# RegulatoryGenomicsGroup/chicdiff

Hardware: AMD Instinct MI355X
Metric: interactions/sec NB-GLM Wald test (higher is better)
Workload: dtype f64; 1 GPU; synthetic 2000000 interactions x 8 samples (4v4), size factors + offsets(theta=0.5) + dispersions + Wald, design ~condition; rows_per_gpu=2000000, samples=8, global_rows=2000000, parallelism=rows-sharded x1, collectives=none (single rank), ranks_in_communicator=1

## Files before the change

chicdiff_amd/csrc/api.hip:

```cpp
#include <math.h>
#include <stdarg.h>
#include <stdio.h>
#include <stdlib.h>
#include <string.h>

#include <algorithm>
#include <mutex>
#include <thread>
#include <string>
#include <vector>
#include <unordered_set>

#include <dlfcn.h>

#include "common.h"
#include "philox.h"
#include "prior_mc.h"

using namespace cd;

namespace cd {
struct ChinputCols {
    std::vector<int32_t> bait, oe, N;
    std::string error;
};
int64_t chinput_parse(const char *path, int nthreads, ChinputCols &c);
}

struct KTimer {
    std::string name;
    hipEvent_t e0 = nullptr, e1 = nullptr;
    double ms = 0;
    int launches = 0;
    double bytes = 0;
};

struct HostOpts {
    int select_all_rounds = 0;
    int trend_one_launch_per_pass = 0;
    int sharded_trend_gather = 1;
    int trend_mad_in_kernel = 1;
    int local_trend_substitute = 1;
    int fuse_offsets = 1;
    int theta_grid_concurrency = 5;
    int host_copy_threads = 12;
    int bench_fake_world = 0;
    int fault_inject = 0;
    int region_assemble_generic = 0;
    int chicago_tables_run_merge = 1;
};

struct chicdiff_hip_ctx {
    int device = 0;
    bool no_persistent_trend = false;
    Opts tune{};
    HostOpts host;
    char *tg_buf = nullptr;
    size_t tg_bytes = 0;
    double shard_n[kSelMaxWorld] = {0};
    bool shard_n_valid = false;
    int64_t tg_total = 0;
    double *tg_x = nullptr, *tg_y = nullptr, *tg_resid = nullptr;
    int32_t *tg_flags = nullptr;
    int32_t *h_flag = nullptr;
    FusedOffsets fuse;
    int refits = 0;
    bool sf_overflow_seen = false;
    int32_t *d_carry = nullptr;
    char *io_dev = nullptr, *io_pin = nullptr;
    size_t io_dev_bytes = 0, io_pin_bytes = 0;
    ChinputCols *chin = nullptr;
    struct EarlyCopy {
        int n = 0;
        struct Item { int col; char *pin; size_t bytes; } item[10];
        hipEvent_t ready = nullptr, done = nullptr;
        bool issued = false;
// ... 9 lines not shown
    void *allgather_user = nullptr;
    int world = 1, rank = 0;
    void *rccl_lib = nullptr, *rccl_comm = nullptr;
    int (*rccl_allreduce)(const void *, void *, size_t, int, int, void *, hipStream_t) = nullptr;
    int (*rccl_allgather)(const void *, void *, size_t, int, void *, hipStream_t) = nullptr;
    int (*rccl_comm_destroy)(void *) = nullptr;
    const char *(*rccl_error_string)(int) = nullptr;
    char err[512] = {0};
    int64_t cap_n = 0;
    int cap_S = 0;
    void *ws = nullptr;
    size_t ws_bytes = 0;
    char *aux = nullptr;
    size_t aux_bytes = 0;
    FitWork w{};
    double *d_sf = nullptr;
    double *d_logfact = nullptr;
    PmcTable *d_pmc[4] = {nullptr, nullptr, nullptr, nullptr};
    double *d_nf_tmp = nullptr;
    unsigned int *d_sfhist = nullptr;
    bool sfhist_dirty = false;
    FitScalars *h_sc = nullptr;
    double *h_sf = nullptr;
    int timing = 0;
    std::vector<KTimer> timers;
    std::vector<std::pair<int, hipEvent_t>> pending;
    std::vector<hipEvent_t> event_pool;
    int scope_depth = 0;
    std::unordered_set<void *> user_allocs;
    std::mutex user_mu;
};

static char g_create_err[512];
constexpr int64_t kFuseOffsetsMaxRows = 1 << 18;

static const PmcTable &pmc_table(int df) {
    static PmcTable tables[4];
    static bool ready[4] = {false, false, false, false};
    static std::mutex mu;
    std::lock_guard<std::mutex> lock(mu);
    if (!ready[df]) {
        pmc_build(df, tables[df]);
        ready[df] = true;
    }
    return tables[df];
}

static int fail(chicdiff_hip_ctx *c, int code, const char *fmt, ...) {
    va_list ap;
    va_start(ap, fmt);
    vsnprintf(c ? c->err : g_create_err, 512, fmt, ap);
    va_end(ap);
    return code;
}
#define HIPCHK(c, call)                                                                              \
    do {                                                                                             \
        hipError_t e_ = (call);                                                                      \
        if (e_ != hipSuccess) return fail(c, CHICDIFF_E_HIP, "%s: %s", #call, hipGetErrorString(e_)); \
    } while (0)

extern "C" {

const char *chicdiff_hip_last_error(const chicdiff_hip_ctx *ctx) { return ctx ? ctx->err : g_create_err; }

void chicdiff_hip_default_opts(chicdiff_nbglm_opts *o) {
    o->minDisp = 1e-8;
    o->dispTol = 1e-6;
// ... 3 lines not shown
    o->betaTol = 1e-8;
    o->minmu = 0.5;
    o->outlierSD = 2.0;
    o->dispPriorVar = NAN;
    o->trendCoef[0] = o->trendCoef[1] = NAN;
    o->fitType = 0;
    o->_pad = 0;
}

struct OptionDef {
    const char *name;
    int32_t Opts::*tune;
    int HostOpts::*host;
    int64_t lo, hi, no_lo, no_hi;
};
static const OptionDef kOptions[] = {
    {"line_search_spread", &Opts::spread, nullptr, 0, 3, 1, 0},
    {"line_search_min_waves", &Opts::min_waves, nullptr, 0, 4, 1, 1},
    {"line_search_chunk", &Opts::chunk, nullptr, 0, 64, 1, 7},
    {"line_search_prio", &Opts::prio, nullptr, 0, 100, 1, 0},
    {"line_search_schedule", &Opts::schedule, nullptr, 0, 4, 2, 2},
    {"line_search_deal", &Opts::deal, nullptr, 0, 64, 1, 0},
    {"line_search_classes_a", &Opts::classes_a, nullptr, 0, 6, 1, 0},
    {"line_search_fillers", &Opts::fillers, nullptr, -1, 1, 1, 0},
    {"line_search_filler_stop", &Opts::filler_stop, nullptr, -1, 100, 1, 0},
    {"theta_grid_concurrency", nullptr, &HostOpts::theta_grid_concurrency, 1, 16, 1, 0},
    {"host_copy_threads", nullptr, &HostOpts::host_copy_threads, 1, 64, 1, 0},
    {"select_all_rounds", nullptr, &HostOpts::select_all_rounds, 0, 1, 1, 0},
    {"trend_one_launch_per_pass", nullptr, &HostOpts::trend_one_launch_per_pass, 0, 1, 1, 0},
    {"sharded_trend_gather", nullptr, &HostOpts::sharded_trend_gather, 0, 1, 1, 0},
    {"trend_persistent_blocks", &Opts::trend_blocks, nullptr, 0, 256, 1, 0},
    {"trend_mad_in_kernel", nullptr, &HostOpts::trend_mad_in_kernel, 0, 1, 1, 0},
    {"fuse_offsets", nullptr, &HostOpts::fuse_offsets, 0, 2, 1, 0},
    {"region_assemble_generic", nullptr, &HostOpts::region_assemble_generic, 0, 1, 1, 0},
    {"chicago_tables_run_merge", nullptr, &HostOpts::chicago_tables_run_merge, 0, 1, 1, 0},
    {"fault_inject", nullptr, &HostOpts::fault_inject, 0, 7, 1, 0},
    {"bench_fake_world", nullptr, &HostOpts::bench_fake_world, 0, kGatherMaxWorld, 1, 0},
    {"local_trend_substitute", nullptr, &HostOpts::local_trend_substitute, 0, 1, 1, 0},
};

int chicdiff_hip_set_option(chicdiff_hip_ctx *c, const char *name, int64_t value) {
    if (!c || !name) return CHICDIFF_E_INVALID;
    for (const OptionDef &d : kOptions) {
        if (strcmp(name, d.name) != 0 || value < d.lo || value > d.hi || (value >= d.no_lo && value <= d.no_hi)) continue;
        if (d.host == &HostOpts::bench_fake_world && value > 1 && !getenv("CHICDIFF_BENCH_FAKE_WORLD"))
            return fail(c, CHICDIFF_E_INVALID, "set_option: bench_fake_world is a rehearsal hook of bench.py (CHICDIFF_BENCH_FAKE_WORLD unset)");
        if (d.tune) c->tune.*d.tune = (int32_t)value;
        else c->host.*d.host = (int)value;
        return CHICDIFF_OK;
    }
    return fail(c, CHICDIFF_E_INVALID, "set_option: unknown option or value (%s = %lld)", name, (long long)value);
}

int chicdiff_hip_create(chicdiff_hip_ctx **out, int32_t device) {
    if (!out) return fail(nullptr, CHICDIFF_E_INVALID, "ctx out pointer is NULL");
    *out = nullptr;
    int ndev = 0;
    hipError_t e = hipGetDeviceCount(&ndev);
    if (e != hipSuccess || ndev <= 0)
        return fail(nullptr, CHICDIFF_E_HIP, "no HIP device available (%s): the HIP path cannot run, and there is no CPU fallback",
                    e != hipSuccess ? hipGetErrorString(e) : "device count 0");
    if (device < 0 || device >= ndev) return fail(nullptr, CHICDIFF_E_INVALID, "device %d out of range [0,%d)", device, ndev);
    chicdiff_hip_ctx *c = new chicdiff_hip_ctx();
    c->device = device;
    if ((e = hipSetDevice(device)) != hipSuccess || (e = hipStreamCreateWithFlags(&c->own_stream, hipStreamNonBlocking)) != hipSuccess ||
        (e = hipHostMalloc((void **)&c->h_sc, sizeof(FitScalars))) != hipSuccess ||
// ... 705 lines not shown
    launch_resid_hist(dm, wm, d_hist, c->stream);
    if (!mad_local)
        if (int rc = do_allreduce(c, d_hist, kPmcBins)) return rc;
    const int df = d.S - d.p;
    if (!c->d_pmc[df]) {
        HIPCHK(c, hipMalloc((void **)&c->d_pmc[df], sizeof(PmcTable)));
        HIPCHK(c, hipMemcpy(c->d_pmc[df], &pmc_table(df), sizeof(PmcTable), hipMemcpyHostToDevice));
    }
    launch_prior_mc(d, c->w, d_hist, c->d_pmc[df], c->stream);
    return CHICDIFF_OK;
}

static int read_scalars(chicdiff_hip_ctx *c) {
    HIPCHK(c, hipMemcpyAsync(c->h_sc, c->w.sc, sizeof(FitScalars), hipMemcpyDeviceToHost, c->stream));
    HIPCHK(c, hipStreamSynchronize(c->stream));
    return CHICDIFF_OK;
}

static int fit_pass(chicdiff_hip_ctx *c, const int32_t *d_counts, const double *d_nf, FitDims d, const Opts &o,
                    const chicdiff_nbglm_out *d_out, bool all_rounds) {
    int rc;
    hipStream_t st = c->stream;
    FitWork &w = c->w;
    c->tg_total = 0;
    HIPCHK(c, hipMemsetAsync(w.sc, 0, align256(sizeof(FitScalars)) + kQueueBytes + 1024, st));
    const int world = c->world > 0 ? c->world : 1;
    const bool col_slots = c->allreduce && world <= kSelMaxWorld;
    const size_t slot_doubles = (size_t)(d.S + 1) * 2;
    double *slots = col_slots ? w.hist : nullptr;
    if (col_slots) HIPCHK(c, hipMemsetAsync(slots, 0, sizeof(double) * slot_doubles * world, st));
    {
        Scope t(c, "prep");
        const bool fused = c->fuse.fm != nullptr && d.S <= 16 && d_nf == c->d_nf_tmp;
        launch_prep(d_counts, const_cast<double *>(d_nf), d, w, o, st, fused ? c->fuse : FusedOffsets());
        launch_prep_finish(d, w, col_slots ? slots + slot_doubles * c->rank : nullptr, st);
    }
    if (col_slots) {
        if ((rc = do_allreduce(c, slots, (int64_t)(slot_doubles * world)))) return rc;
    } else if ((rc = do_allreduce(c, w.sc->colsum, kMaxS + 1)))
        return rc;
    if (c->allreduce) launch_xim(d, w, slots, world, st);
    {
        Scope t(c, "disp_gene");
        Opts og = o;
        og.xim_here = c->allreduce ? 0 : 1;
        launch_disp_gene(d_counts, d_nf, d, w, og, st);
    }
    bool mad_in_kernel = false;
    if (o.trendIn[0] == o.trendIn[0] && o.trendIn[1] == o.trendIn[1]) {
        launch_trend_init(d, w, o, st);
        HIPCHK(c, hipMemcpyAsync(w.sc->coefs, o.trendIn, sizeof(double) * 2, hipMemcpyHostToDevice, st));
        HIPCHK(c, hipStreamSynchronize(st));
    } else if (o.fit_type == 1) {
        if (c->allreduce) return fail(c, CHICDIFF_E_INVALID, "fitType \"mean\" is not available for sharded fits");
        std::vector<double> g((size_t)d.n);
        HIPCHK(c, hipMemcpyAsync(g.data(), w.dispGene, sizeof(double) * (size_t)d.n, hipMemcpyDeviceToHost, st));
        HIPCHK(c, hipStreamSynchronize(st));
        size_t m = 0;
        for (size_t i = 0; i < g.size(); i++)
            if (g[i] > 10 * o.minDisp) g[m++] = g[i];
        if (m == 0) return fail(c, CHICDIFF_E_NUMERIC, "fitType \"mean\": no gene-wise estimate above 10 * minDisp");
        const size_t lo = (size_t)floor((double)m * 0.001), hi = m - lo;
        if (lo > 0) {
            std::nth_element(g.begin(), g.begin() + lo, g.begin() + m);
            std::nth_element(g.begin() + lo, g.begin() + (hi - 1), g.begin() + m);
        }
        long double acc = 0;
        for (size_t i = lo; i < hi; i++) acc += g[i];
// ... 123 lines not shown
        } else
            break;
        c->refits++;
    }
    if (scalars) {
        const FitScalars *s = c->h_sc;
        int status = 0;
        if (s->failed) status |= CHICDIFF_ST_TREND_FAILED;
        if (s->trend_local) status |= CHICDIFF_ST_TREND_LOCAL;
        scalars->trendCoef[0] = s->coefs[0];
        scalars->trendCoef[1] = s->coefs[1];
        scalars->varLogDispEsts = s->varLogDispEsts;
        scalars->dispPriorVar = s->dispPriorVar;
        scalars->nAllZero = (int64_t)hs[2];
        scalars->sumDeviance = hs[2] > 0 ? NAN : hs[0];
        scalars->trendOuterIter = s->outer_it;
        if (hs[2] > 0) status |= CHICDIFF_ST_ALLZERO_ROWS;
        if (hs[1] > 0) status |= CHICDIFF_ST_BETA_NONCONV;
        if (prior_by_simulation(d, o)) status |= CHICDIFF_ST_PRIORVAR_MC;
        scalars->status = status;
    }
    return CHICDIFF_OK;
}

static int begin_call(chicdiff_hip_ctx *c, int rc, int64_t n, int32_t S) {
    timing_reset(c);
    if ((rc = shard_consensus(c, rc, n))) return rc;
    HIPCHK(c, hipSetDevice(c->device));
    if ((rc = ensure_workspace(c, n, S))) return rc;
    c->refits = 0;
    return CHICDIFF_OK;
}

static void form_offsets(chicdiff_hip_ctx *c, const double *d_fullMean, int64_t n, int32_t S, double theta, int mix) {
    if (d_fullMean && S <= 16 && c->host.fuse_offsets && (c->host.fuse_offsets == 2 || n <= kFuseOffsetsMaxRows)) {
        c->fuse.fm = d_fullMean;
        c->fuse.sf = c->d_sf;
        c->fuse.theta = theta;
        c->fuse.mix = mix;
    } else {
        Scope t(c, "offsets");
        launch_offsets(d_fullMean, c->d_sf, n, S, theta, mix, c->d_nf_tmp, c->stream);
    }
}

extern "C" {

int chicdiff_hip_nbglm_fit_dev(chicdiff_hip_ctx *c, const int32_t *d_counts, const double *d_nf, int64_t n, int32_t S,
                               const int32_t *group, const chicdiff_nbglm_opts *opts, const chicdiff_nbglm_out *d_out,
                               chicdiff_nbglm_scalars *scalars) {
    if (!c) return CHICDIFF_E_INVALID;
    FitDims d;
    int rc = (!d_counts || !d_nf) ? fail(c, CHICDIFF_E_INVALID, "counts / nf pointer is NULL") : check_counts_group(c, n, S, group, d);
    if (!rc) rc = check_opts(c, opts);
    if ((rc = begin_call(c, rc, n, S))) return rc;
    HIPCHK(c, hipMemsetAsync(c->d_carry, 0, sizeof(int32_t), c->stream));
    rc = fit_dev_impl(c, d_counts, d_nf, d, make_opts(c, opts, S), d_out, scalars, c->host.select_all_rounds != 0);
    timing_collect(c);
    return rc;
}

static int ensure_io(chicdiff_hip_ctx *c, size_t dev_bytes, size_t pin_bytes) {
    if (c->io_dev_bytes < dev_bytes) {
        if (c->io_dev) { HIPCHK(c, hipStreamSynchronize(c->stream)); (void)hipFree(c->io_dev); c->io_dev = nullptr; c->io_dev_bytes = 0; }
        hipError_t e = hipMalloc((void **)&c->io_dev, dev_bytes);
        if (e != hipSuccess) return fail(c, CHICDIFF_E_NOMEM, "device arena of %zu bytes: %s", dev_bytes, hipGetErrorString(e));
        c->io_dev_bytes = dev_bytes;
    }
// ... 1049 lines not shown
```

chicdiff_amd/csrc/common.h:

```cpp
#pragma once
#include <hip/hip_runtime.h>
#include <stdint.h>

#include "../../include/chicdiff_hip.h"
#include "fit_driver.h"
#include "fit_state.h"

namespace cd {

constexpr int kRedBlocks = 1024;

struct FitDims {
    int64_t n;
    int32_t S, p, nA, nB;
    uint64_t gmask;
};

struct FitWork {
    double *baseMean, *baseVar, *gm0, *gm1, *rough, *binit0, *binit1, *crow;
    double *dispGene, *dispFit, *dispMAP, *disp, *beta0, *beta1, *resid;
    int32_t *allZero, *geneIter, *mapIter, *outlier, *betaIter, *optimConv;
    int32_t *order;
    uint8_t *cls;
    int32_t *gridlist;
// ... 87 lines not shown
    if (a == 4) return kSchedMinDispSlot;
    if (a == 5) return (mode == kSchedSix || mode == kSchedMinDispLast) ? kSchedClassesFine - 1 : kSchedMinDispSlot;
    return kSchedClassesFine;
}
#ifdef __HIPCC__
template <int NC>
__device__ __forceinline__ void order_hist_store(const unsigned int (&mine)[NC], unsigned int *hist) {
    __shared__ unsigned int s_cnt[NC];
    if (threadIdx.x < NC) s_cnt[threadIdx.x] = 0;
    __syncthreads();
#pragma unroll
    for (int k = 0; k < NC; k++) {
        unsigned int v = mine[k];
        for (int off = 32; off > 0; off >>= 1) v += __shfl_down(v, off);
        if ((threadIdx.x & 63) == 0 && v) atomicAdd(&s_cnt[k], v);
    }
    __syncthreads();
    if (threadIdx.x < NC) hist[threadIdx.x * kSchedBlocks + blockIdx.x] = s_cnt[threadIdx.x];
}
__device__ __forceinline__ void class_peers(int c, bool valid, int lane, unsigned int &rank, unsigned int &count) {
    unsigned long long m = __ballot(valid);
#pragma unroll
    for (int b = 0; b < 5; b++) {
        const bool bit = (c >> b) & 1;
        const unsigned long long set = __ballot(bit);
        m &= bit ? set : ~set;
    }
    rank = __popcll(m & ((1ull << lane) - 1ull));
    count = __popcll(m);
}
#endif

struct FusedOffsets { const double *fm = nullptr; const double *sf = nullptr; double theta = 0; int mix = 0; };
void launch_prep(const int32_t *counts, double *nf, FitDims d, FitWork w, Opts o, hipStream_t st, FusedOffsets fo = FusedOffsets());
void launch_prep_finish(FitDims d, FitWork w, double *slot, hipStream_t st);
void launch_xim(FitDims d, FitWork w, const double *slots, int world, hipStream_t st);
void launch_disp_gene(const int32_t *counts, const double *nf, FitDims d, FitWork w, Opts o, hipStream_t st);
void launch_order_build(FitDims d, FitWork w, int classesA, bool have_hist, hipStream_t st, bool fine = false);
void launch_disp_map(const int32_t *counts, const double *nf, FitDims d, FitWork w, Opts o, hipStream_t st);
void launch_trend_persistent(FitDims d, FitWork w, Opts o, hipStream_t st, bool with_mad);
int trend_persistent_blocks();
void launch_trend_init(FitDims d, FitWork w, Opts o, hipStream_t st);
int trend_blocks();
void launch_trend_pass(FitDims d, FitWork w, Opts o, hipStream_t st, bool fused_step);
void launch_trend_step(FitDims d, FitWork w, Opts o, hipStream_t st);
constexpr int kLfMaxV = 100;
struct LfVerts { int nv; int _pad; double x[kLfMaxV], f[kLfMaxV], d[kLfMaxV]; };
void launch_lf_hist(FitDims d, FitWork w, Opts o, int use_dist, double xv, uint64_t prefix, int shift, double *hist, hipStream_t st);
void launch_lf_sums(FitDims d, FitWork w, Opts o, double xv, double h, double *partials, double *out8, hipStream_t st);
void launch_lf_eval(FitDims d, FitWork w, const LfVerts &v, hipStream_t st);
void launch_trend_gather(FitDims d, FitWork w, Opts o, double *xg, double *yg, hipStream_t st);
constexpr int kGatherMaxWorld = 64;
struct GatherLayout { int32_t world, _pad; int64_t block, maxn; int64_t off[kGatherMaxWorld + 1]; };
void launch_trend_compact(const GatherLayout &gl, const double *recv, double *xg, double *yg, hipStream_t st);
void launch_poke(int32_t *p, int32_t v, hipStream_t st);
void launch_flag_to_double(const int32_t *flag, double *out, hipStream_t st);
void launch_dispfit_resid(FitDims d, FitWork w, Opts o, hipStream_t st);
void launch_prior_var(FitDims d, FitWork w, Opts o, hipStream_t st);
void launch_resid_hist(FitDims d, FitWork w, double *out40, hipStream_t st);
void launch_prior_mc(FitDims d, FitWork w, const double *hist40, const void *table, hipStream_t st);
void launch_wald_prep(const int32_t *counts, const double *nf, FitDims d, FitWork w, Opts o, hipStream_t st);
void launch_wald_irls(const int32_t *counts, const double *nf, FitDims d, FitWork w, Opts o, hipStream_t st);
void launch_wald_final(const int32_t *counts, const double *nf, FitDims d, FitWork w, Opts o,
                       const chicdiff_nbglm_out &out, hipStream_t st);
void launch_wald_intercept(const int32_t *counts, const double *nf, FitDims d, FitWork w, Opts o,
                           const chicdiff_nbglm_out &out, hipStream_t st);
void launch_dev_sum_finish(FitDims d, FitWork w, const int32_t *carry, const double *sf_dev, hipStream_t st);

// ... 151 lines not shown
```

chicdiff_amd/csrc/devmath.h:

```cpp
#pragma once
#include <hip/hip_runtime.h>

#include "exp_table.h"
#include "fit_state.h"
#include "log_table.h"

namespace cd {

__device__ __forceinline__ double fma3(double a, double b, double c) {
    double d;
    asm("v_fma_f64 %0, %1, %2, %3" : "=v"(d) : "v"(a), "v"(b), "v"(c));
    return d;
}

__device__ __forceinline__ double rcp(double x) {
    double r = __builtin_amdgcn_rcp(x);
    double e = fma(-x, r, 1.0);
    r = fma(r, e, r);
    e = fma(-x, r, 1.0);
    return fma(r, e, r);
}

__device__ __forceinline__ double rcp_or_div(double x) { return (x > 1e-300 && x < 1e300) ? rcp(x) : 1.0 / x; }

// ... 237 lines not shown
        const double temp = y * (xnum + 18154.981253343561249) / (xden + 45507.789335026729956);
        return 2.0 * (0.5 - temp);
    }
    double temp;
    if (y <= 5.656854249492380195206754896838) {
        double xnum = 1.0765576773720192317e-8 * y, xden = y;
        xnum = (xnum + 0.39894151208813466764) * y;  xden = (xden + 22.266688044328115691) * y;
        xnum = (xnum + 8.8831497943883759412) * y;   xden = (xden + 235.38790178262499861) * y;
        xnum = (xnum + 93.506656132177855979) * y;   xden = (xden + 1519.377599407554805) * y;
        xnum = (xnum + 597.27027639480026226) * y;   xden = (xden + 6485.558298266760755) * y;
        xnum = (xnum + 2494.5375852903726711) * y;   xden = (xden + 18615.571640885098091) * y;
        xnum = (xnum + 6848.1904505362823326) * y;   xden = (xden + 34900.952721145977266) * y;
        xnum = (xnum + 11602.651437647350124) * y;   xden = (xden + 38912.003286093271411) * y;
        temp = (xnum + 9842.7148383839780218) / (xden + 19685.429676859990727);
    } else if (y < 37.5193) {
        const double xsq = 1.0 / (y * y);
        double xnum = 0.02307344176494017303 * xsq, xden = xsq;
        xnum = (xnum + 0.21589853405795699) * xsq;      xden = (xden + 1.28426009614491121) * xsq;
        xnum = (xnum + 0.1274011611602473639) * xsq;    xden = (xden + 0.468238212480865118) * xsq;
        xnum = (xnum + 0.022235277870649807) * xsq;     xden = (xden + 0.0659881378689285515) * xsq;
        xnum = (xnum + 0.001421619193227893466) * xsq;  xden = (xden + 0.00378239633202758244) * xsq;
        temp = xsq * (xnum + 2.9112874951168792e-5) / (xden + 7.29751555083966205e-5);
        temp = (0.398942280401432677939946059934 - temp) / y;
    } else {
        return 0.0;
    }
    const double xsq = trunc(y * 16) / 16;
    const double del = (y - xsq) * (y + xsq);
    return 2.0 * (exp(-xsq * xsq * 0.5) * exp(-del * 0.5) * temp);
}


__device__ __forceinline__ double rlog_t(double x, const LogEntry *lt) { return (x > 2.3e-308 && x < 1.7e308) ? tlog(x, lt) : log(x); }
__device__ __forceinline__ void offsets_row16(double (&v)[16], int S, const double *__restrict__ sf, double theta, int mix, const LogEntry *lt) {
    const double iS = 1.0 / S;
    double sl = 0;
#pragma unroll
    for (int j = 0; j < 16; j++)
        if (j < S) sl += rlog_t(v[j], lt);
    const double gmean = exp(sl * iS);
    const double ig = (gmean > 1e-300 && gmean < 1e300) ? rcp(gmean) : 1.0 / gmean;
    bool anyna = false;
#pragma unroll
    for (int j = 0; j < 16; j++)
        if (j < S) {
            v[j] = v[j] * ig;
            anyna |= (v[j] != v[j]);
        }
    double sl2 = 0;
#pragma unroll
    for (int j = 0; j < 16; j++)
        if (j < S) {
            if (anyna) v[j] = sf[j];
            if (mix) {
                v[j] = v[j] * (1 - theta) + sf[j] * theta;
                sl2 += rlog_t(v[j], lt);
            }
        }
    if (mix) {
        const double g2 = exp(sl2 * iS);
        const double i2 = (g2 > 1e-300 && g2 < 1e300) ? rcp(g2) : 1.0 / g2;
#pragma unroll
        for (int j = 0; j < 16; j++)
            if (j < S) v[j] = v[j] * i2;
    }
}

}
```

chicdiff_amd/csrc/disp_kernels.hip:

```cpp
#include <stdio.h>
#include <stdlib.h>

#include <vector>

#include "common.h"
#include "devmath.h"

namespace cd {

struct DD { double hi, lo; };
__device__ __forceinline__ void dd_add(DD &a, double x) {
    const double s = a.hi + x, bb = s - a.hi;
    a.lo += (a.hi - (s - bb)) + (x - bb);
    a.hi = s;
}
__device__ __forceinline__ void dd_add(DD &a, const DD &b) {
    dd_add(a, b.hi);
    a.lo += b.lo;
    const double s = a.hi + a.lo;
    a.lo = a.lo - (s - a.hi);
    a.hi = s;
}

struct CountProfile { unsigned int w0 = 0, w1 = 0, w2 = 0; };
__device__ __forceinline__ void profile_add(CountProfile &c, int y) {
    const unsigned int m = (unsigned int)(y < 10 ? y : 10);
    const unsigned int a = m < 4u ? m : 4u, b = m < 4u ? 0u : (m < 8u ? m - 4u : 4u), d = m < 8u ? 0u : m - 8u;
    c.w0 += 0x01010101u & (a == 4u ? 0xffffffffu : ((1u << (8u * a)) - 1u));
    c.w1 += 0x01010101u & (b == 4u ? 0xffffffffu : ((1u << (8u * b)) - 1u));
    c.w2 += 0x00000101u & ((1u << (8u * d)) - 1u);
}
__device__ __forceinline__ void prep_store(FitDims d, FitWork w, int64_t i, double s, double g0, double g1, double v,
                                           double est, int64_t tot) {
    w.baseMean[i] = s / d.S;
    w.baseVar[i] = v / (d.S - 1);
    w.gm0[i] = g0;
    w.gm1[i] = g1;
    w.rough[i] = fmax(est / (d.S - d.p), 0.0);
    w.allZero[i] = (tot == 0);
}

template <bool FUSED>
__global__ __launch_bounds__(256) void prep16_kernel(const int32_t *__restrict__ counts,
                                                     double *__restrict__ nf, FitDims d, FitWork w, FusedOffsets fo) {
    __shared__ LogEntry s_lt[FUSED ? 64 : 1];
    if (FUSED) log_table_to_lds(s_lt);
    extern __shared__ uint32_t s_tile[];
    __shared__ DD s_part[256];
    __shared__ unsigned char s_live[256];
    const int T = blockDim.x;
    const int64_t n = d.n;
    const int S = d.S;
    const int64_t stride = row_stride(S);
    const int ldw = (int)(stride / 4) + 1, qpr = (int)(stride / 16);
    const int tid = threadIdx.x;
    const int ncol = S + 1, G = T / ncol, cg = tid / ncol, cc = tid % ncol;
    DD colacc{0.0, 0.0};
    for (int64_t base = (int64_t)blockIdx.x * T; base < n; base += (int64_t)gridDim.x * T) {
        const int64_t i = base + tid;
        const int nrows = n - base < T ? (int)(n - base) : T;
        if (i < n) {
            double q[16];
            double s = 0, g0 = 0, g1 = 0;
            int64_t tot = 0;
            int32_t sign = 0;
            CountProfile cprof;
            uint32_t *row = s_tile + tid * ldw;
            row[7] = 0;
            for (int k = 8 + 3 * S; k < (int)(stride / 4); k++) row[k] = 0;
            double fv[16];
            if (FUSED) {
#pragma unroll
                for (int j = 0; j < 16; j++) fv[j] = j < S ? fo.fm[(int64_t)j * n + i] : 1.0;
                offsets_row16(fv, S, fo.sf, fo.theta, fo.mix, s_lt);
#pragma unroll
                for (int j = 0; j < 16; j++)
                    if (j < S) nf[(int64_t)j * n + i] = fv[j];
            }
#pragma unroll
            for (int j = 0; j < 16; j++) {
                q[j] = 0;
                if (j < S) {
                    const int32_t k = counts[(int64_t)j * n + i];
                    const double f = FUSED ? fv[j] : nf[(int64_t)j * n + i];
                    row[8 + 2 * j] = (uint32_t)__double2loint(f);
                    row[8 + 2 * j + 1] = (uint32_t)__double2hiint(f);
                    row[8 + 2 * S + j] = (uint32_t)k;
                    profile_add(cprof, k);
                    sign |= k;
                    q[j] = (double)k / f;
                    tot += k;
                    s += q[j];
                    if ((d.gmask >> j) & 1) g1 += q[j]; else g0 += q[j];
                }
            }
            const double bm = s / S;
            g0 /= d.nA;
            if (d.p == 2) g1 /= d.nB;
            row[0] = (uint32_t)__double2loint(g0);
            row[1] = (uint32_t)__double2hiint(g0) | (tot == 0 ? 0x80000000u : 0u);
            row[2] = (uint32_t)__double2loint(g1);
            row[3] = (uint32_t)__double2hiint(g1);
            row[4] = cprof.w0;
            row[5] = cprof.w1;
            row[6] = cprof.w2;
            s_live[tid] = tot != 0;
            const double m0 = fmax(1.0, g0), m1 = fmax(1.0, g1);
            const double i0 = 1.0 / (m0 * m0), i1 = 1.0 / (m1 * m1);
            double v = 0, est = 0;
#pragma unroll
            for (int j = 0; j < 16; j++)
                if (j < S) {
                    v += (q[j] - bm) * (q[j] - bm);
                    const bool g = (d.gmask >> j) & 1;
                    const double mj = g ? m1 : m0;
                    est += ((q[j] - mj) * (q[j] - mj) - mj) * (g ? i1 : i0);
                }
            prep_store(d, w, i, s, g0, g1, v, est, tot);
            if (sign < 0) w.sc->neg_counts = 1;
        }
        __syncthreads();
        uint4 *dst = reinterpret_cast<uint4 *>(w.rowpack + base * stride);
        for (int c = tid; c < nrows * qpr; c += T) {
            const uint32_t *src = s_tile + (c / qpr) * ldw + (c % qpr) * 4;
            dst[c] = make_uint4(src[0], src[1], src[2], src[3]);
        }
        if (cg < G) {
            DD a{0.0, 0.0};
            for (int r = cg; r < nrows; r += G)
                if (s_live[r]) {
                    const uint32_t *src = s_tile + r * ldw + 8 + 2 * cc;
                    dd_add(a, cc < S ? __hiloint2double((int)src[1], (int)src[0]) : 1.0);
                }
            s_part[cg * ncol + cc] = a;
        }
        __syncthreads();
        if (tid < ncol)
            for (int g = 0; g < G; g++) dd_add(colacc, s_part[g * ncol + tid]);
        __syncthreads();
    }
    if (tid < ncol) {
        w.partials[((int64_t)tid * gridDim.x + blockIdx.x) * 2] = colacc.hi;
        w.partials[((int64_t)tid * gridDim.x + blockIdx.x) * 2 + 1] = colacc.lo;
    }
}

__global__ __launch_bounds__(256) void prep_kernel(const int32_t *__restrict__ counts,
                                                   const double *__restrict__ nf, FitDims d, FitWork w) {
    const int64_t n = d.n;
    const int S = d.S;
    for (int64_t i = blockIdx.x * (int64_t)blockDim.x + threadIdx.x; i < n; i += (int64_t)gridDim.x * blockDim.x) {
        double s = 0, g0 = 0, g1 = 0;
        int64_t tot = 0;
        double *rp_nf = reinterpret_cast<double *>(w.rowpack + i * row_stride(S) + kRowHdr);
        int32_t *rp_y = reinterpret_cast<int32_t *>(rp_nf + S);
        CountProfile cprof;
        for (int j = 0; j < S; j++) {
            const int32_t k = counts[(int64_t)j * n + i];
            if (k < 0) w.sc->neg_counts = 1;
            profile_add(cprof, k);
            rp_nf[j] = nf[(int64_t)j * n + i];
            rp_y[j] = k;
            const double q = (double)k / nf[(int64_t)j * n + i];
            tot += k;
            s += q;
            if ((d.gmask >> j) & 1) g1 += q; else g0 += q;
        }
        const double bm = s / S;
        g0 /= d.nA;
        if (d.p == 2) g1 /= d.nB;
        reinterpret_cast<double2 *>(row_hdr(w.rowpack, i, S))[0] = make_double2(tot == 0 ? -0.0 : g0, g1);
        reinterpret_cast<uint4 *>(row_hdr(w.rowpack, i, S))[1] = make_uint4(cprof.w0, cprof.w1, cprof.w2, 0u);
        const double m0 = fmax(1.0, g0), m1 = fmax(1.0, g1);
        double v = 0, est = 0;
        for (int j = 0; j < S; j++) {
            const double q = (double)counts[(int64_t)j * n + i] / nf[(int64_t)j * n + i];
// ... 30 lines not shown
        for (int off = 32; off > 0; off >>= 1) dd_add(a, DD{__shfl_down(a.hi, off), __shfl_down(a.lo, off)});
    } else {
        double s = 0;
        for (int b = lane; b < nblk; b += 64) s += w.partials[(int64_t)j * nblk + b];
        for (int off = 32; off > 0; off >>= 1) s += __shfl_down(s, off);
        a.hi = s;
    }
    if (lane == 0) {
        if (slot) {
            slot[2 * j] = a.hi;
            slot[2 * j + 1] = a.lo;
        } else {
            const double s = a.hi + a.lo;
            if (j < d.S) w.sc->colsum[j] = s; else w.sc->nnz = s;
        }
    }
}

__global__ void xim_kernel(FitDims d, FitWork w, const double *slots, int world) {
    if (threadIdx.x || blockIdx.x) return;
    if (slots)
        for (int j = 0; j <= d.S; j++) {
            DD a{0.0, 0.0};
            for (int r = 0; r < world; r++) dd_add(a, DD{slots[((size_t)r * (d.S + 1) + j) * 2], slots[((size_t)r * (d.S + 1) + j) * 2 + 1]});
            const double s = a.hi + a.lo;
            if (j < d.S) w.sc->colsum[j] = s; else w.sc->nnz = s;
        }
    double x = 0;
    for (int j = 0; j < d.S; j++) x += 1.0 / (w.sc->colsum[j] / w.sc->nnz);
    w.sc->xim = x / d.S;
}

constexpr int kColsumBlocks = 512;
static int prep16_blocks(int) { return 1024; }
void launch_prep(const int32_t *counts, double *nf, FitDims d, FitWork w, Opts, hipStream_t st, FusedOffsets fo) {
    if (d.S <= 16) {
        const int T = row_stride(d.S) > 128 ? 128 : 256;
        if (fo.fm) prep16_kernel<true><<<prep16_blocks(d.S), T, (size_t)T * (row_stride(d.S) + 4), st>>>(counts, nf, d, w, fo);
        else prep16_kernel<false><<<prep16_blocks(d.S), T, (size_t)T * (row_stride(d.S) + 4), st>>>(counts, nf, d, w, fo);
    } else {
        prep_kernel<<<kRedBlocks, 256, 0, st>>>(counts, nf, d, w);
        colsum_kernel<<<dim3(kColsumBlocks, d.S + 1), 256, 0, st>>>(nf, d, w);
    }
}
void launch_prep_finish(FitDims d, FitWork w, double *slot, hipStream_t st) {
    colsum_finish_kernel<<<d.S + 1, 64, 0, st>>>(d, w, d.S <= 16 ? prep16_blocks(d.S) : kColsumBlocks, d.S <= 16, slot);
}
void launch_xim(FitDims d, FitWork w, const double *slots, int world, hipStream_t st) { xim_kernel<<<1, 64, 0, st>>>(d, w, slots, world); }

constexpr int kSchedClassesA = 2, kSchedDeal = 8;
template <int NC>
__global__ __launch_bounds__(256) void order_hist_kernel(const uint8_t *__restrict__ cls, int64_t n, int64_t tile, unsigned int *hist) {
    const int64_t lo = (int64_t)blockIdx.x * tile, hi = lo + tile < n ? lo + tile : n;
    unsigned int mine[NC] = {};
    for (int64_t i = lo + threadIdx.x; i < hi; i += 256) {
        const int c = cls[i];
#pragma unroll
        for (int k = 0; k < NC; k++) mine[k] += (c == k);
    }
    order_hist_store<NC>(mine, hist);
}
template <int NC>
__global__ __launch_bounds__(256) void order_scatter_kernel(const uint8_t *__restrict__ cls, int64_t n, int64_t tile,
                                                            const unsigned int *__restrict__ hist, int32_t *__restrict__ order,
                                                            FitScalars *sc, int classesA, int classesB) {
    static_assert(NC <= 32 && kSchedBlocks == 4 * 256, "8 threads per class sum 256 partial counts; class_peers() tells 32 classes apart");
    __shared__ unsigned int s_m[NC][256];
    __shared__ unsigned int s_edge[NC];
    __shared__ unsigned int s_part[NC][8][2];
    __shared__ unsigned int s_tot[NC], s_pre[NC];
    __shared__ unsigned int s_wh[4][NC];
    __shared__ unsigned int s_wbase[4][NC];
    const int nblk = gridDim.x, t = threadIdx.x, lane = t & 63, wave = t >> 6, blk = blockIdx.x;
    if (t < 4 * NC) (&s_wh[0][0])[t] = 0;
    __syncthreads();
    const int64_t lo = (int64_t)blk * tile, hi = lo + tile < n ? lo + tile : n;
    const int64_t quarter = tile / 4;
    const int64_t wlo = lo + wave * quarter, whi = wlo + quarter < hi ? wlo + quarter : hi;
    for (int64_t i0 = wlo; i0 < whi; i0 += 64) {
// ... 805 lines not shown
```

chicdiff_amd/csrc/global_kernels.hip:

```cpp
#include "common.h"
#include "devmath.h"
#include "prior_mc.h"

namespace cd {

template <int K>
__device__ __forceinline__ void block_reduce_store(double (&v)[K], double *out) {
    __shared__ double red[K][4];
    const int lane = threadIdx.x & 63, wave = threadIdx.x >> 6;
#pragma unroll
    for (int k = 0; k < K; k++) {
        double x = v[k];
        for (int off = 32; off > 0; off >>= 1) x += __shfl_down(x, off);
        if (lane == 0) red[k][wave] = x;
    }
    __syncthreads();
    if (threadIdx.x < K) out[threadIdx.x] = (red[threadIdx.x][0] + red[threadIdx.x][1]) + (red[threadIdx.x][2] + red[threadIdx.x][3]);
}

__global__ void reduce_partials_kernel(const double *partials, int nblk, int K, double *sums) {
    __shared__ double red[256];
    for (int k = 0; k < K; k++) {
        double acc = 0;
        for (int b = threadIdx.x; b < nblk; b += 256) acc += partials[(int64_t)b * K + k];
// ... 1446 lines not shown
            double rk[2] = {rank0, 0};
            sf_list_select(list, a.n, false, m0, nb, b0, 1, rk, s_h, s_c, &s_nc, s_res);
            rk[0] = rank1;
            sf_list_select(list, a.n, true, m1, nb, b1, 1, rk, s_h, s_c, &s_nc, s_res + 1);
        }
    }
    __syncthreads();
    if (threadIdx.x == 0) {
        sc->sel_prefix[2 * col] = s_res[0];
        sc->sel_prefix[2 * col + 1] = s_res[1];
        if (col == 0) sc->sel_fast_done = 1;
        sel_finish_col(a, sc, col);
    }
}

void launch_sf_direct(const int32_t *counts, int64_t n, int S, SelArgs a, FitWork w, unsigned int *hist, uint64_t *lists,
                      int32_t *clear_flag, int cus, hipStream_t st) {
    const int nb = sf_bins(S);
    int64_t hb = (n + kSfThreads - 1) / kSfThreads;
    if (hb > (cus > 0 ? cus : 256)) hb = cus > 0 ? cus : 256;
    unsigned int *gcnt = hist + kSfHistWords;
    if (S <= 4) sf_hist_kernel<4><<<(unsigned)hb, kSfThreads, 0, st>>>(counts, n, S, nb, hist, clear_flag);
    else if (S <= 8) sf_hist_kernel<8><<<(unsigned)hb, kSfThreads, 0, st>>>(counts, n, S, nb, hist, clear_flag);
    else sf_hist_kernel<16><<<(unsigned)hb, kSfThreads, 0, st>>>(counts, n, S, nb, hist, clear_flag);
    sf_pick_kernel<<<S, kSfThreads, 0, st>>>(w, hist, gcnt, nb);
    if (S <= 4) sf_list_kernel<4><<<(unsigned)hb, kSfThreads, 0, st>>>(counts, n, S, nb, w, gcnt, lists);
    else if (S <= 8) sf_list_kernel<8><<<(unsigned)hb, kSfThreads, 0, st>>>(counts, n, S, nb, w, gcnt, lists);
    else sf_list_kernel<16><<<(unsigned)hb, kSfThreads, 0, st>>>(counts, n, S, nb, w, gcnt, lists);
    sf_finish_kernel<<<S, kSfThreads, 0, st>>>(a, w, nb, gcnt, lists);
}

__device__ __forceinline__ double rlog(double x) { return (x > 0.0 && x < 1.7e308) ? flog(x) : log(x); }

__global__ __launch_bounds__(256) void offsets16_kernel(const double *__restrict__ fm, const double *__restrict__ sf,
                                                        int64_t n, int S, double theta, int mix,
                                                        double *__restrict__ out) {
    __shared__ LogEntry s_lt[64];
    log_table_to_lds(s_lt);
    for (int64_t i = blockIdx.x * 256 + threadIdx.x; i < n; i += (int64_t)gridDim.x * 256) {
        double v[16];
#pragma unroll
        for (int j = 0; j < 16; j++) v[j] = j < S ? fm[(int64_t)j * n + i] : 1.0;
        offsets_row16(v, S, sf, theta, mix, s_lt);
#pragma unroll
        for (int j = 0; j < 16; j++)
            if (j < S) out[(int64_t)j * n + i] = v[j];
    }
}

__global__ __launch_bounds__(256) void offsets_kernel(const double *__restrict__ fm, const double *__restrict__ sf,
                                                      int64_t n, int S, double theta, int mix,
                                                      double *__restrict__ out) {
    for (int64_t i = blockIdx.x * 256 + threadIdx.x; i < n; i += (int64_t)gridDim.x * 256) {
        double sl = 0;
        for (int j = 0; j < S; j++) sl += rlog(fm[(int64_t)j * n + i]);
        const double gmean = exp(sl / S);
        bool anyna = false;
        for (int j = 0; j < S; j++) {
            const double m3 = fm[(int64_t)j * n + i] / gmean;
            anyna |= (m3 != m3);
        }
        double g2 = 1.0;
        if (mix) {
            double sl2 = 0;
            for (int j = 0; j < S; j++) {
                const double m3 = anyna ? sf[j] : fm[(int64_t)j * n + i] / gmean;
                sl2 += rlog(m3 * (1 - theta) + sf[j] * theta);
            }
            g2 = exp(sl2 / S);
        }
        for (int j = 0; j < S; j++) {
            double m3 = anyna ? sf[j] : fm[(int64_t)j * n + i] / gmean;
            if (mix) m3 = (m3 * (1 - theta) + sf[j] * theta) / g2;
            out[(int64_t)j * n + i] = m3;
        }
    }
}
__global__ __launch_bounds__(256) void offsets_sf_kernel(const double *__restrict__ sf, int64_t n, int S, double *__restrict__ out) {
    for (int64_t i = blockIdx.x * 256 + threadIdx.x; i < n; i += (int64_t)gridDim.x * 256)
        for (int j = 0; j < S; j++) out[(int64_t)j * n + i] = sf[j];
}
void launch_offsets(const double *fm, const double *sf_dev, int64_t n, int S, double theta, int mix, double *out,
                    hipStream_t st) {
    int64_t blocks = (n + 255) / 256;
    if (blocks > 4096) blocks = 4096;
    if (!fm) {
        offsets_sf_kernel<<<(unsigned)blocks, 256, 0, st>>>(sf_dev, n, S, out);
        return;
    }
    if (S <= 16)
        offsets16_kernel<<<(unsigned)blocks, 256, 0, st>>>(fm, sf_dev, n, S, theta, mix, out);
    else
        offsets_kernel<<<(unsigned)blocks, 256, 0, st>>>(fm, sf_dev, n, S, theta, mix, out);
}

constexpr int kWinCap = 256 * 12;
__global__ __launch_bounds__(256) void window_sums_kernel(const int32_t *__restrict__ fragN,
                                                          const double *__restrict__ fragFM, int64_t nfrag, int S,
                                                          const int64_t *__restrict__ rptr, int64_t n,
                                                          int32_t *__restrict__ N, double *__restrict__ FM) {
    __shared__ int32_t s_n[kWinCap];
    __shared__ double s_f[kWinCap];
    const int j = blockIdx.y;
    const int64_t nblk = (n + 255) / 256;
    for (int64_t blk = blockIdx.x; blk < nblk; blk += gridDim.x) {
        const int64_t i0 = blk * 256, i1 = (i0 + 256 < n) ? i0 + 256 : n;
        const int64_t f0 = rptr[i0], f1 = rptr[i1];
        const int64_t i = i0 + threadIdx.x;
        const bool staged = (f1 - f0) <= kWinCap;
        int64_t lo = 0, hi = 0;
        if (i < i1) { lo = rptr[i]; hi = rptr[i + 1]; }
        if (staged) {
            __syncthreads();
            const int span = (int)(f1 - f0);
            if (fragN) {
                int32_t v[12];
#pragma unroll
                for (int k = 0; k < 12; k++) {
                    const int e = threadIdx.x + k * 256;
                    v[k] = e < span ? fragN[(int64_t)j * nfrag + f0 + e] : 0;
                }
#pragma unroll
                for (int k = 0; k < 12; k++) {
                    const int e = threadIdx.x + k * 256;
// ... 685 lines not shown
```

Before: 584.8 million interactions/s.

## Specialize prep kernel by sample count, prefetch next rows, size grid to residency

The prep kernel is now templated on padded sample count (4/8/16), so S=8 uses 8-wide register arrays instead of 16. It software-prefetches the next grid-stride iteration's counts and means into registers before the tile store. The grid is sized from occupancy × CU count instead of a fixed 1024 blocks. Fused offset formation is also enabled for all row counts (the 2^18 row cap is removed), the per-block column accumulator moves to shared memory, and the finish kernel receives the actual block count. Together these aim to cut memory latency stalls and the separate offsets pass, at the cost of more registers per thread and more template instantiations.

```diff
diff --git a/chicdiff_amd/csrc/api.hip b/chicdiff_amd/csrc/api.hip
--- a/chicdiff_amd/csrc/api.hip
+++ b/chicdiff_amd/csrc/api.hip
@@ -42,6 +42,7 @@
     int trend_mad_in_kernel = 1;
     int local_trend_substitute = 1;
     int fuse_offsets = 1;
+    int prep_blocks = 0;
     int theta_grid_concurrency = 5;
     int host_copy_threads = 12;
     int bench_fake_world = 0;
@@ -117,7 +118,6 @@
 };
 
 static char g_create_err[512];
-constexpr int64_t kFuseOffsetsMaxRows = 1 << 18;
 
 static const PmcTable &pmc_table(int df) {
     static PmcTable tables[4];
@@ -187,6 +187,7 @@
     {"trend_persistent_blocks", &Opts::trend_blocks, nullptr, 0, 256, 1, 0},
     {"trend_mad_in_kernel", nullptr, &HostOpts::trend_mad_in_kernel, 0, 1, 1, 0},
     {"fuse_offsets", nullptr, &HostOpts::fuse_offsets, 0, 2, 1, 0},
+    {"prep_blocks", nullptr, &HostOpts::prep_blocks, 0, kRedBlocks, 1, 0},
     {"region_assemble_generic", nullptr, &HostOpts::region_assemble_generic, 0, 1, 1, 0},
     {"chicago_tables_run_merge", nullptr, &HostOpts::chicago_tables_run_merge, 0, 1, 1, 0},
     {"fault_inject", nullptr, &HostOpts::fault_inject, 0, 7, 1, 0},
@@ -958,8 +959,8 @@
     {
         Scope t(c, "prep");
         const bool fused = c->fuse.fm != nullptr && d.S <= 16 && d_nf == c->d_nf_tmp;
-        launch_prep(d_counts, const_cast<double *>(d_nf), d, w, o, st, fused ? c->fuse : FusedOffsets());
-        launch_prep_finish(d, w, col_slots ? slots + slot_doubles * c->rank : nullptr, st);
+        const int nblk = launch_prep(d_counts, const_cast<double *>(d_nf), d, w, o, st, fused ? c->fuse : FusedOffsets(), c->host.prep_blocks);
+        launch_prep_finish(d, w, nblk, col_slots ? slots + slot_doubles * c->rank : nullptr, st);
     }
     if (col_slots) {
         if ((rc = do_allreduce(c, slots, (int64_t)(slot_doubles * world)))) return rc;
@@ -1149,8 +1150,9 @@
     return CHICDIFF_OK;
 }
 
+static bool fused_offsets_win(int64_t, int32_t S) { return S <= 16; }
 static void form_offsets(chicdiff_hip_ctx *c, const double *d_fullMean, int64_t n, int32_t S, double theta, int mix) {
-    if (d_fullMean && S <= 16 && c->host.fuse_offsets && (c->host.fuse_offsets == 2 || n <= kFuseOffsetsMaxRows)) {
+    if (d_fullMean && S <= 16 && c->host.fuse_offsets && (c->host.fuse_offsets == 2 || fused_offsets_win(n, S))) {
         c->fuse.fm = d_fullMean;
         c->fuse.sf = c->d_sf;
         c->fuse.theta = theta;
diff --git a/chicdiff_amd/csrc/common.h b/chicdiff_amd/csrc/common.h
--- a/chicdiff_amd/csrc/common.h
+++ b/chicdiff_amd/csrc/common.h
@@ -143,8 +143,8 @@
 #endif
 
 struct FusedOffsets { const double *fm = nullptr; const double *sf = nullptr; double theta = 0; int mix = 0; };
-void launch_prep(const int32_t *counts, double *nf, FitDims d, FitWork w, Opts o, hipStream_t st, FusedOffsets fo = FusedOffsets());
-void launch_prep_finish(FitDims d, FitWork w, double *slot, hipStream_t st);
+int launch_prep(const int32_t *counts, double *nf, FitDims d, FitWork w, Opts o, hipStream_t st, FusedOffsets fo = FusedOffsets(), int max_blocks = 0);
+void launch_prep_finish(FitDims d, FitWork w, int nblk, double *slot, hipStream_t st);
 void launch_xim(FitDims d, FitWork w, const double *slots, int world, hipStream_t st);
 void launch_disp_gene(const int32_t *counts, const double *nf, FitDims d, FitWork w, Opts o, hipStream_t st);
 void launch_order_build(FitDims d, FitWork w, int classesA, bool have_hist, hipStream_t st, bool fine = false);
diff --git a/chicdiff_amd/csrc/devmath.h b/chicdiff_amd/csrc/devmath.h
--- a/chicdiff_amd/csrc/devmath.h
+++ b/chicdiff_amd/csrc/devmath.h
@@ -293,24 +293,25 @@
 
 
 __device__ __forceinline__ double rlog_t(double x, const LogEntry *lt) { return (x > 2.3e-308 && x < 1.7e308) ? tlog(x, lt) : log(x); }
-__device__ __forceinline__ void offsets_row16(double (&v)[16], int S, const double *__restrict__ sf, double theta, int mix, const LogEntry *lt) {
+template <int N>
+__device__ __forceinline__ void offsets_row16(double (&v)[N], int S, const double *__restrict__ sf, double theta, int mix, const LogEntry *lt) {
     const double iS = 1.0 / S;
     double sl = 0;
 #pragma unroll
-    for (int j = 0; j < 16; j++)
+    for (int j = 0; j < N; j++)
         if (j < S) sl += rlog_t(v[j], lt);
     const double gmean = exp(sl * iS);
     const double ig = (gmean > 1e-300 && gmean < 1e300) ? rcp(gmean) : 1.0 / gmean;
     bool anyna = false;
 #pragma unroll
-    for (int j = 0; j < 16; j++)
+    for (int j = 0; j < N; j++)
         if (j < S) {
             v[j] = v[j] * ig;
             anyna |= (v[j] != v[j]);
         }
     double sl2 = 0;
 #pragma unroll
-    for (int j = 0; j < 16; j++)
+    for (int j = 0; j < N; j++)
         if (j < S) {
             if (anyna) v[j] = sf[j];
             if (mix) {
@@ -322,7 +323,7 @@
         const double g2 = exp(sl2 * iS);
         const double i2 = (g2 > 1e-300 && g2 < 1e300) ? rcp(g2) : 1.0 / g2;
 #pragma unroll
-        for (int j = 0; j < 16; j++)
+        for (int j = 0; j < N; j++)
             if (j < S) v[j] = v[j] * i2;
     }
 }
diff --git a/chicdiff_amd/csrc/disp_kernels.hip b/chicdiff_amd/csrc/disp_kernels.hip
--- a/chicdiff_amd/csrc/disp_kernels.hip
+++ b/chicdiff_amd/csrc/disp_kernels.hip
@@ -40,56 +40,71 @@
     w.allZero[i] = (tot == 0);
 }
 
-template <bool FUSED>
-__global__ __launch_bounds__(256) void prep16_kernel(const int32_t *__restrict__ counts,
-                                                     double *__restrict__ nf, FitDims d, FitWork w, FusedOffsets fo) {
+template <int N, typename V>
+__device__ __forceinline__ void prep16_load(const V *__restrict__ src, int64_t n, int S, int64_t i, V (&v)[N]) {
+    const int64_t ii = i < n ? i : 0;
+#pragma unroll
+    for (int j = 0; j < N; j++) v[j] = src[(int64_t)(j < S ? j : S - 1) * n + ii];
+}
+
+template <bool FUSED, int N>
+__global__ __launch_bounds__(N == 16 ? 128 : 256, N == 16 ? 2 : 4) void prep16_kernel(const int32_t *__restrict__ counts,
+                                                                                      double *__restrict__ nf, FitDims d, FitWork w, FusedOffsets fo) {
     __shared__ LogEntry s_lt[FUSED ? 64 : 1];
-    if (FUSED) log_table_to_lds(s_lt);
+    __shared__ double s_sf[FUSED ? 16 : 1];
+    if (FUSED) {
+        if ((int)threadIdx.x < d.S) s_sf[threadIdx.x] = fo.sf[threadIdx.x];
+        log_table_to_lds(s_lt);
+    }
     extern __shared__ uint32_t s_tile[];
     __shared__ DD s_part[256];
     __shared__ unsigned char s_live[256];
-    const int T = blockDim.x;
+    constexpr int T = N == 16 ? 128 : 256;
     const int64_t n = d.n;
     const int S = d.S;
     const int64_t stride = row_stride(S);
     const int ldw = (int)(stride / 4) + 1, qpr = (int)(stride / 16);
     const int tid = threadIdx.x;
-    const int ncol = S + 1, G = T / ncol, cg = tid / ncol, cc = tid % ncol;
-    DD colacc{0.0, 0.0};
-    for (int64_t base = (int64_t)blockIdx.x * T; base < n; base += (int64_t)gridDim.x * T) {
+    const int ncol = S + 1, G = T / ncol;
+    __shared__ DD s_col[17];
+    if (tid < ncol) s_col[tid] = DD{0.0, 0.0};
+    const double *__restrict__ src = FUSED ? fo.fm : nf;
+    int32_t kv[N];
+    double fv[N];
+    uint32_t *row = s_tile + tid * ldw;
+    row[7] = 0;
+    for (int k = 8 + 3 * S; k < (int)(stride / 4); k++) row[k] = 0;
+    int64_t base = (int64_t)blockIdx.x * T;
+    prep16_load<N>(src, n, S, base + tid, fv);
+    if (!FUSED) prep16_load<N>(counts, n, S, base + tid, kv);
+    while (base < n) {
         const int64_t i = base + tid;
+        const int64_t next = base + (int64_t)gridDim.x * T;
         const int nrows = n - base < T ? (int)(n - base) : T;
         if (i < n) {
-            double q[16];
+            double q[N];
             double s = 0, g0 = 0, g1 = 0;
-            int64_t tot = 0;
             int32_t sign = 0;
             CountProfile cprof;
-            uint32_t *row = s_tile + tid * ldw;
-            row[7] = 0;
-            for (int k = 8 + 3 * S; k < (int)(stride / 4); k++) row[k] = 0;
-            double fv[16];
             if (FUSED) {
+                offsets_row16<N>(fv, S, s_sf, fo.theta, fo.mix, s_lt);
+                prep16_load<N>(counts, n, S, i, kv);
 #pragma unroll
-                for (int j = 0; j < 16; j++) fv[j] = j < S ? fo.fm[(int64_t)j * n + i] : 1.0;
-                offsets_row16(fv, S, fo.sf, fo.theta, fo.mix, s_lt);
+                for (int j = 0; j < N; j++)
+                    if (j < S) nf[(int64_t)j * n + i] = fv[j];
+            }
 #pragma unroll
-                for (int j = 0; j < 16; j++)
-                    if (j < S) nf[(int64_t)j * n + i] = fv[j];
-            }
-#pragma unroll
-            for (int j = 0; j < 16; j++) {
+            for (int j = 0; j < N; j++) {
                 q[j] = 0;
                 if (j < S) {
-                    const int32_t k = counts[(int64_t)j * n + i];
-                    const double f = FUSED ? fv[j] : nf[(int64_t)j * n + i];
+                    const int32_t k = kv[j];
+                    const double f = fv[j];
                     row[8 + 2 * j] = (uint32_t)__double2loint(f);
                     row[8 + 2 * j + 1] = (uint32_t)__double2hiint(f);
                     row[8 + 2 * S + j] = (uint32_t)k;
                     profile_add(cprof, k);
                     sign |= k;
                     q[j] = (double)k / f;
-                    tot += k;
                     s += q[j];
                     if ((d.gmask >> j) & 1) g1 += q[j]; else g0 += q[j];
                 }
@@ -98,33 +113,36 @@
             g0 /= d.nA;
             if (d.p == 2) g1 /= d.nB;
             row[0] = (uint32_t)__double2loint(g0);
-            row[1] = (uint32_t)__double2hiint(g0) | (tot == 0 ? 0x80000000u : 0u);
+            row[1] = (uint32_t)__double2hiint(g0) | (sign == 0 ? 0x80000000u : 0u);
             row[2] = (uint32_t)__double2loint(g1);
             row[3] = (uint32_t)__double2hiint(g1);
             row[4] = cprof.w0;
             row[5] = cprof.w1;
             row[6] = cprof.w2;
-            s_live[tid] = tot != 0;
+            s_live[tid] = sign != 0;
             const double m0 = fmax(1.0, g0), m1 = fmax(1.0, g1);
             const double i0 = 1.0 / (m0 * m0), i1 = 1.0 / (m1 * m1);
             double v = 0, est = 0;
 #pragma unroll
-            for (int j = 0; j < 16; j++)
+            for (int j = 0; j < N; j++)
                 if (j < S) {
                     v += (q[j] - bm) * (q[j] - bm);
                     const bool g = (d.gmask >> j) & 1;
                     const double mj = g ? m1 : m0;
                     est += ((q[j] - mj) * (q[j] - mj) - mj) * (g ? i1 : i0);
                 }
-            prep_store(d, w, i, s, g0, g1, v, est, tot);
+            prep_store(d, w, i, s, g0, g1, v, est, sign != 0);
             if (sign < 0) w.sc->neg_counts = 1;
         }
+        prep16_load<N>(src, n, S, next + tid, fv);
+        if (!FUSED) prep16_load<N>(counts, n, S, next + tid, kv);
         __syncthreads();
         uint4 *dst = reinterpret_cast<uint4 *>(w.rowpack + base * stride);
         for (int c = tid; c < nrows * qpr; c += T) {
             const uint32_t *src = s_tile + (c / qpr) * ldw + (c % qpr) * 4;
             dst[c] = make_uint4(src[0], src[1], src[2], src[3]);
         }
+        const int cg = tid / ncol, cc = tid % ncol;
         if (cg < G) {
             DD a{0.0, 0.0};
             for (int r = cg; r < nrows; r += G)
@@ -135,13 +153,17 @@
             s_part[cg * ncol + cc] = a;
         }
         __syncthreads();
-        if (tid < ncol)
+        if (tid < ncol) {
+            DD colacc = s_col[tid];
             for (int g = 0; g < G; g++) dd_add(colacc, s_part[g * ncol + tid]);
+            s_col[tid] = colacc;
+        }
         __syncthreads();
+        base = next;
     }
     if (tid < ncol) {
-        w.partials[((int64_t)tid * gridDim.x + blockIdx.x) * 2] = colacc.hi;
-        w.partials[((int64_t)tid * gridDim.x + blockIdx.x) * 2 + 1] = colacc.lo;
+        w.partials[((int64_t)tid * gridDim.x + blockIdx.x) * 2] = s_col[tid].hi;
+        w.partials[((int64_t)tid * gridDim.x + blockIdx.x) * 2 + 1] = s_col[tid].lo;
     }
 }
 
@@ -238,19 +260,47 @@
 }
 
 constexpr int kColsumBlocks = 512;
-static int prep16_blocks(int) { return 1024; }
-void launch_prep(const int32_t *counts, double *nf, FitDims d, FitWork w, Opts, hipStream_t st, FusedOffsets fo) {
+template <bool FUSED, int N>
+static int prep16_resident() {
+    static const int blocks = [] {
+        constexpr int T = N == 16 ? 128 : 256;
+        int per_cu = 0, dev = 0, cus = 0;
+        if (hipOccupancyMaxActiveBlocksPerMultiprocessor(&per_cu, prep16_kernel<FUSED, N>, T, (size_t)T * (row_stride(N) + 4)) != hipSuccess || per_cu < 1 || per_cu > 4) per_cu = 4;
+        if (hipGetDevice(&dev) != hipSuccess || hipDeviceGetAttribute(&cus, hipDeviceAttributeMultiprocessorCount, dev) != hipSuccess || cus < 1) cus = 256;
+        (void)hipGetLastError();
+        const int b = per_cu * cus;
+        return b < kRedBlocks ? b : kRedBlocks;
+    }();
+    return blocks;
+}
+template <bool FUSED>
+static int prep16_blocks(int S) { return S <= 4 ? prep16_resident<FUSED, 4>() : S <= 8 ? prep16_resident<FUSED, 8>() : prep16_resident<FUSED, 16>(); }
+template <bool FUSED, int N>
+static void prep16_launch(int blocks, const int32_t *counts, double *nf, FitDims d, FitWork w, hipStream_t st, FusedOffsets fo) {
+    constexpr int T = N == 16 ? 128 : 256;
+    prep16_kernel<FUSED, N><<<blocks, T, (size_t)T * (row_stride(d.S) + 4), st>>>(counts, nf, d, w, fo);
+}
+int launch_prep(const int32_t *counts, double *nf, FitDims d, FitWork w, Opts, hipStream_t st, FusedOffsets fo, int max_blocks) {
     if (d.S <= 16) {
-        const int T = row_stride(d.S) > 128 ? 128 : 256;
-        if (fo.fm) prep16_kernel<true><<<prep16_blocks(d.S), T, (size_t)T * (row_stride(d.S) + 4), st>>>(counts, nf, d, w, fo);
-        else prep16_kernel<false><<<prep16_blocks(d.S), T, (size_t)T * (row_stride(d.S) + 4), st>>>(counts, nf, d, w, fo);
-    } else {
-        prep_kernel<<<kRedBlocks, 256, 0, st>>>(counts, nf, d, w);
-        colsum_kernel<<<dim3(kColsumBlocks, d.S + 1), 256, 0, st>>>(nf, d, w);
-    }
-}
-void launch_prep_finish(FitDims d, FitWork w, double *slot, hipStream_t st) {
-    colsum_finish_kernel<<<d.S + 1, 64, 0, st>>>(d, w, d.S <= 16 ? prep16_blocks(d.S) : kColsumBlocks, d.S <= 16, slot);
+        int blocks = fo.fm ? prep16_blocks<true>(d.S) : prep16_blocks<false>(d.S);
+        if (max_blocks > 0 && max_blocks < blocks) blocks = max_blocks;
+        if (fo.fm) {
+            if (d.S <= 4) prep16_launch<true, 4>(blocks, counts, nf, d, w, st, fo);
+            else if (d.S <= 8) prep16_launch<true, 8>(blocks, counts, nf, d, w, st, fo);
+            else prep16_launch<true, 16>(blocks, counts, nf, d, w, st, fo);
+        } else {
+            if (d.S <= 4) prep16_launch<false, 4>(blocks, counts, nf, d, w, st, fo);
+            else if (d.S <= 8) prep16_launch<false, 8>(blocks, counts, nf, d, w, st, fo);
+            else prep16_launch<false, 16>(blocks, counts, nf, d, w, st, fo);
+        }
+        return blocks;
+    }
+    prep_kernel<<<kRedBlocks, 256, 0, st>>>(counts, nf, d, w);
+    colsum_kernel<<<dim3(kColsumBlocks, d.S + 1), 256, 0, st>>>(nf, d, w);
+    return kColsumBlocks;
+}
+void launch_prep_finish(FitDims d, FitWork w, int nblk, double *slot, hipStream_t st) {
+    colsum_finish_kernel<<<d.S + 1, 64, 0, st>>>(d, w, nblk, d.S <= 16, slot);
 }
 void launch_xim(FitDims d, FitWork w, const double *slots, int world, hipStream_t st) { xim_kernel<<<1, 64, 0, st>>>(d, w, slots, world); }
 
diff --git a/chicdiff_amd/csrc/global_kernels.hip b/chicdiff_amd/csrc/global_kernels.hip
--- a/chicdiff_amd/csrc/global_kernels.hip
+++ b/chicdiff_amd/csrc/global_kernels.hip
@@ -1502,18 +1502,19 @@
 
 __device__ __forceinline__ double rlog(double x) { return (x > 0.0 && x < 1.7e308) ? flog(x) : log(x); }
 
+template <int N>
 __global__ __launch_bounds__(256) void offsets16_kernel(const double *__restrict__ fm, const double *__restrict__ sf,
                                                         int64_t n, int S, double theta, int mix,
                                                         double *__restrict__ out) {
     __shared__ LogEntry s_lt[64];
     log_table_to_lds(s_lt);
     for (int64_t i = blockIdx.x * 256 + threadIdx.x; i < n; i += (int64_t)gridDim.x * 256) {
-        double v[16];
-#pragma unroll
-        for (int j = 0; j < 16; j++) v[j] = j < S ? fm[(int64_t)j * n + i] : 1.0;
-        offsets_row16(v, S, sf, theta, mix, s_lt);
-#pragma unroll
-        for (int j = 0; j < 16; j++)
+        double v[N];
+#pragma unroll
+        for (int j = 0; j < N; j++) v[j] = j < S ? fm[(int64_t)j * n + i] : 1.0;
+        offsets_row16<N>(v, S, sf, theta, mix, s_lt);
+#pragma unroll
+        for (int j = 0; j < N; j++)
             if (j < S) out[(int64_t)j * n + i] = v[j];
     }
 }
@@ -1558,8 +1559,12 @@
         offsets_sf_kernel<<<(unsigned)blocks, 256, 0, st>>>(sf_dev, n, S, out);
         return;
     }
-    if (S <= 16)
-        offsets16_kernel<<<(unsigned)blocks, 256, 0, st>>>(fm, sf_dev, n, S, theta, mix, out);
+    if (S <= 4)
+        offsets16_kernel<4><<<(unsigned)blocks, 256, 0, st>>>(fm, sf_dev, n, S, theta, mix, out);
+    else if (S <= 8)
+        offsets16_kernel<8><<<(unsigned)blocks, 256, 0, st>>>(fm, sf_dev, n, S, theta, mix, out);
+    else if (S <= 16)
+        offsets16_kernel<16><<<(unsigned)blocks, 256, 0, st>>>(fm, sf_dev, n, S, theta, mix, out);
     else
         offsets_kernel<<<(unsigned)blocks, 256, 0, st>>>(fm, sf_dev, n, S, theta, mix, out);
 }
```

Measured after the change: 591.5 million interactions/s (median of 6 runs). 1.1% higher.
